# adrianstanea/UnitSpeech

Measured on AMD Instinct MI355X. Metric: mel-frames/sec @ 50 diffusion steps, 80x1024, higher is better.
Workload: dtype f32; 1 GPU; B=1 utterance(s)/GPU, 80x1024 mel, 50 diffusion steps, text+spk CFG (3 score evals/step), full-size decoder (119.1M params, synthetic weights), built-in Philox noise; batch_per_gpu=1, frames=1024, diffusion_steps=50, parallelism=utterance-sharded x1

## Files before the change

unitspeech_amd/csrc/conv_igemm.hip:

```cpp
#include <type_traits>
#include "kernels.h"
#include "pack_f16.h"

namespace us {

typedef float f32x4 __attribute__((ext_vector_type(4)));
typedef _Float16 half8 __attribute__((ext_vector_type(8)));

constexpr int TN = 128;

__device__ __forceinline__ void blds16(__amdgpu_buffer_rsrc_t rsrc, unsigned voff_bytes, unsigned soff_bytes, float* lds_dst_wave_uniform) {
  __builtin_amdgcn_raw_ptr_buffer_load_lds(rsrc, (__attribute__((address_space(3))) void*)lds_dst_wave_uniform, 16, (int)voff_bytes,
                                           (int)soff_bytes, 0, 0);
}

template <int BK, int WM, bool WINO, bool F16 = false, int NWM = 2, int NSTG = 2, bool ASPLIT = false, int NB = 2>
__global__ __launch_bounds__(NWM * 128, 2) void conv_igemm_kernel(ConvArgs a) {
  constexpr int TN = 64 * NB;
  constexpr int NW = 2 * NWM;
  constexpr int TM = NWM * WM;
  constexpr int MB = WM / 32;
  constexpr int CPR = BK / 4;
  constexpr int RPI = 64 / CPR;
  constexpr int IA = TM / RPI / NW;
  constexpr int IB = TN / RPI / NW;
  static_assert(NSTG == 2 || NSTG == 3, "two or three operand buffers");
  constexpr int SWZ_DIV = 64 / BK;
  constexpr int BUF = (TM + TN) * BK;
  extern __shared__ __attribute__((aligned(16))) float smem[];

  const int tid = threadIdx.x, lane = tid & 63;
  const int wave = __builtin_amdgcn_readfirstlane(tid >> 6);
  const int wm = wave >> 1, wn = wave & 1;
#ifdef US_LIFE
  unsigned long long life_t[5];
#define US_LIFE_AT(i) asm volatile("s_memrealtime %0\n\ts_waitcnt lgkmcnt(0)" : "=s"(life_t[i])::"memory")
  US_LIFE_AT(0);
#endif
  const int l32 = lane & 31, hh = lane >> 5;
  int bt = (int)blockIdx.x, bz = (int)blockIdx.z;
  const bool xcd_z = a.xcd_z && ((gridDim.x * gridDim.z) & 7u) == 0;
  if (xcd_z) {
    const unsigned lin = blockIdx.x + gridDim.x * blockIdx.z;
    const unsigned lp = (lin & 7u) * ((gridDim.x * gridDim.z) >> 3) + (lin >> 3);
    bz = (int)(lp / gridDim.x);
    bt = (int)(lp - (unsigned)bz * gridDim.x);
  }
  const int phase = a.nphase > 1 ? bz % a.nphase : 0;
  const int b = a.nphase > 1 ? bz / a.nphase : bz;
  const unsigned long long dy_bits = a.nphase > 1 ? a.ph_dy[phase] : a.dy_bits, dx_bits = a.nphase > 1 ? a.ph_dx[phase] : a.dx_bits,
                           wtap_bits = a.nphase > 1 ? a.ph_wtap[phase] : a.wtap_bits;
  const int a_oy0 = a.nphase > 1 ? (phase >> 1) : a.oy0, a_ox0 = a.nphase > 1 ? (phase & 1) : a.ox0;
  if (!xcd_z && (gridDim.x & 7u) == 0) bt = (bt & 7) * (int)(gridDim.x >> 3) + (bt >> 3);
  const int bx = bt / a.nt;
  const int ks = a.ksplit > 1 ? bx % a.ksplit : 0;
  const int m0 = (a.ksplit > 1 ? bx / a.ksplit : bx) * TM, n0 = (bt - bx * a.nt) * TN;
  const int Ms = a.Hs * a.Ws;
  const int nchunk = a.Cin / BK;
  const int S_all = a.ntaps * nchunk;
  const int s_lo = a.ksplit > 1 ? (int)(((long long)S_all * ks) / a.ksplit) : 0;
  const int S = a.ksplit > 1 ? (int)(((long long)S_all * (ks + 1)) / a.ksplit) - s_lo : S_all;

  const int lrow = lane / CPR, lpos = lane % CPR;
  int my[IA], mx[IA], achunk[IA];
  bool mv[IA];
#pragma unroll
  for (int j = 0; j < IA; ++j) {
    const int r = (wave * IA + j) * RPI + lrow;
    const int m = m0 + r;
    mv[j] = m < Ms;
    const int mc = mv[j] ? m : 0;
    my[j] = mc / a.Ws;
    mx[j] = mc - my[j] * a.Ws;
    achunk[j] = (lpos ^ ((r / SWZ_DIV) % CPR)) * 4;
  }
  unsigned boff[IB];
#pragma unroll
  for (int j = 0; j < IB; ++j) {
    const int r = (wave * IB + j) * RPI + lrow;
    int n = n0 + r;
    n = n < a.Cout ? n : a.Cout - 1;
    boff[j] = (unsigned)(n * BK + (lpos ^ ((r / SWZ_DIV) % CPR)) * 4) * 4u;
  }
  const unsigned a_bytes = (unsigned)a.Hin * (unsigned)a.Win * (unsigned)a.in_ld * 4u;
  const long long a_item = (long long)a.Hin * a.Win * a.in_ld;
  __amdgpu_buffer_rsrc_t rsrc_a = __builtin_amdgcn_make_buffer_rsrc((void*)(a.in + (long long)b * a_item), 0, (int)a_bytes, 0x00020000);
  __amdgpu_buffer_rsrc_t rsrc_b = __builtin_amdgcn_make_buffer_rsrc(
      (void*)(a.wt + (WINO ? 0LL : (long long)(a.wt_bdiv > 1 ? b / a.wt_bdiv : b) * a.wt_bstride)), 0, 0x7fffffff, 0x00020000);

  unsigned aoff[IA];
// ... 542 lines not shown
        stat_add(a.stats, b, n / cg, 0, bx, (double)s1);
        stat_add(a.stats, b, n / cg, 1, bx, (double)s2);
      }
    }
  }
#ifdef US_LIFE
  US_LIFE_AT(4);
  US_LIFE_AT(3);
  if (a.stamp_out && lane == 0) {
    unsigned long long* o = a.stamp_out + ((blockIdx.x + gridDim.x * blockIdx.z) * NW + wave) * 4;
    o[0] = life_t[0]; o[1] = life_t[1]; o[2] = life_t[2]; o[3] = life_t[3];
  }
#endif
}

__global__ __launch_bounds__(256) void splitk_finish_kernel(ConvArgs a) {
  __shared__ double s_g[kGroups][2];
  const int b = blockIdx.y;
  const int Ms = a.Hs * a.Ws;
  const int C4 = a.Cout >> 2;
  const long long total = (long long)Ms * C4;
  if (threadIdx.x < kGroups * 2) s_g[threadIdx.x >> 1][threadIdx.x & 1] = 0.0;
  __syncthreads();
  float t1[4] = {0.f, 0.f, 0.f, 0.f}, t2[4] = {0.f, 0.f, 0.f, 0.f};
  int tn = -1;
  const bool dense = (a.ostep == 1 && a.oy0 == 0 && a.ox0 == 0 && a.Hs == a.Hout && a.Ws == a.Wout);
  const float alpha = a.alpha ? *a.alpha : 1.f;
  float* out_b = a.out + (long long)b * a.Hout * a.Wout * a.out_ld;
  const float* add_b = a.add ? a.add + (long long)b * a.Hout * a.Wout * a.add_ld : nullptr;
  const float* om_b = a.omask ? a.omask + (long long)(b % a.omask_bmod) * a.omask_ld : nullptr;
  const long long slice = (long long)a.B * Ms * a.Cout;
  const int cg = a.Cout / kGroups;
  for (long long i = blockIdx.x * 256LL + threadIdx.x; i < total; i += (long long)gridDim.x * 256) {
    const int n = (int)(i % C4) * 4;
    const int m = (int)(i / C4);
    const float* p = a.splitk_ws + ((long long)b * Ms + m) * a.Cout + n;
    f32x4 v = *reinterpret_cast<const f32x4*>(p);
    int k = 1;
    for (; k + 8 <= a.ksplit; k += 8) {
      f32x4 u[8];
#pragma unroll
      for (int j = 0; j < 8; ++j) u[j] = *reinterpret_cast<const f32x4*>(p + (k + j) * slice);
#pragma unroll
      for (int j = 0; j < 8; ++j) v += u[j];
    }
    for (; k < a.ksplit; ++k) v += *reinterpret_cast<const f32x4*>(p + k * slice);
    if (a.bias) v += *reinterpret_cast<const f32x4*>(a.bias + n);
    if (a.stats) {
      if (tn >= 0 && tn != n) {
#pragma unroll
        for (int k = 0; k < 4; ++k) {
          atomicAdd(&s_g[(tn + k) / cg][0], (double)t1[k]);
          atomicAdd(&s_g[(tn + k) / cg][1], (double)t2[k]);
          t1[k] = t2[k] = 0.f;
        }
      }
      tn = n;
#pragma unroll
      for (int k = 0; k < 4; ++k) { t1[k] += v[k]; t2[k] += v[k] * v[k]; }
    }
    const int yy = m / a.Ws, xx = m - yy * a.Ws;
    const int ox = a.ox0 + xx * a.ostep;
    const long long pix = dense ? (long long)m : (long long)(a.oy0 + yy * a.ostep) * a.Wout + ox;
    if (a.out2) *reinterpret_cast<f32x4*>(a.out2 + ((long long)b * a.Hout * a.Wout + pix) * a.out2_ld + n) = v;
    v *= alpha;
    if (add_b) v += *reinterpret_cast<const f32x4*>(add_b + pix * a.add_ld + n);
    if (om_b) v *= om_b[ox * a.omask_step];
    *reinterpret_cast<f32x4*>(out_b + pix * a.out_ld + n) = v;
  }
  if (a.stats) {
    if (tn >= 0) {
#pragma unroll
      for (int k = 0; k < 4; ++k) {
        atomicAdd(&s_g[(tn + k) / cg][0], (double)t1[k]);
        atomicAdd(&s_g[(tn + k) / cg][1], (double)t2[k]);
      }
    }
    __syncthreads();
    if (threadIdx.x < kGroups * 2)
      stat_add(a.stats, b, threadIdx.x >> 1, threadIdx.x & 1, blockIdx.x, s_g[threadIdx.x >> 1][threadIdx.x & 1]);
  }
}

static size_t lds_bytes(int bk, int tm, int nstg = 2, int tn = TN) { return (size_t)nstg * (tm + tn) * bk * sizeof(float); }

template <int BK, int WM, bool WINO, bool F16 = false, int NWM = 2, int NSTG = 2, bool ASPLIT = false>
static hipError_t set_attr() {
  return hipFuncSetAttribute(reinterpret_cast<const void*>(&conv_igemm_kernel<BK, WM, WINO, F16, NWM, NSTG, ASPLIT>),
                             hipFuncAttributeMaxDynamicSharedMemorySize, (int)lds_bytes(BK, NWM * WM, NSTG));
}

hipError_t conv_igemm_init() {
  hipError_t e;
  if ((e = set_attr<32, 64, false>()) != hipSuccess) return e;
  if ((e = set_attr<32, 32, false>()) != hipSuccess) return e;
  if ((e = set_attr<16, 64, false>()) != hipSuccess) return e;
  if ((e = set_attr<16, 32, false>()) != hipSuccess) return e;
  if ((e = set_attr<32, 32, true>()) != hipSuccess) return e;
  if ((e = set_attr<32, 64, false, true>()) != hipSuccess) return e;
  if ((e = set_attr<32, 64, false, true, 4, 3>()) != hipSuccess) return e;
  if ((e = hipFuncSetAttribute(reinterpret_cast<const void*>(&conv_igemm_kernel<32, 64, false, true, 4, 3, false, 1>),
                               hipFuncAttributeMaxDynamicSharedMemorySize, (int)lds_bytes(32, 256, 3, 64))) != hipSuccess) return e;
  if ((e = set_attr<32, 64, false, true, 4, 3, true>()) != hipSuccess) return e;
  if ((e = set_attr<32, 64, false, true, 2, 2, true>()) != hipSuccess) return e;
  if ((e = set_attr<32, 32, false, true, 2, 2, true>()) != hipSuccess) return e;
  if ((e = set_attr<32, 32, false, true>()) != hipSuccess) return e;
  if ((e = set_attr<32, 32, true, true, 2, 3>()) != hipSuccess) return e;
  return set_attr<16, 32, true>();
}

hipError_t launch_conv_igemm(const ConvArgs& a_in, hipStream_t s) {
  ConvArgs a = a_in;
  a.range_flag = current_range_flag();
  if (a.B <= 0 || a.Hs <= 0 || a.Ws <= 0) return hipSuccess;
  if (!a.in || !a.wt || !a.out) return hipErrorInvalidValue;
  if ((a.bk != 16 && a.bk != 32) || a.Cin % a.bk != 0 || a.ntaps < 1 || a.ntaps > kMaxTaps) return hipErrorInvalidValue;
  if (a.in_ld % 4 != 0) return hipErrorInvalidValue;
  if (a.Cout % 4 != 0 || a.out_ld % 4 != 0 || (a.add && a.add_ld % 4 != 0)) return hipErrorInvalidValue;
  if ((long long)a.Hin * a.Win * a.in_ld * 4 >= (1LL << 31) || (long long)kMaxTaps * a.Cout * a.Cin * 4 >= (1LL << 31))
    return hipErrorInvalidValue;
  if (a.stats) {
    int cg = a.Cout / kGroups;
    if (a.Cout % kGroups != 0 || (cg & (cg - 1)) != 0) return hipErrorInvalidValue;
  }
  if (a.out2 && (a.out2_ld % 4 != 0 || a.wino_out || a.out_split || a.attn_part_ctx)) return hipErrorInvalidValue;
  const int Ms = a.Hs * a.Ws;
  int tn = TN;
  int nt = (a.Cout + TN - 1) / TN;
  int tm = a.tm;
  if (a.f16) {
    if (a.bk != 32) return hipErrorInvalidValue;
    if (a.f16 == 1 && !a.direct_presplit && a.ntaps == 1 && a.istride == 1 && !a.bias && !a.add) a.splitk_ws = nullptr;
    if (tm == 0) {
      if (a.f16 == 1 && (a.ntaps > 1 || a.direct_presplit)) {
        tm = (a.ntaps == 1 && a.nphase <= 1) || (long long)a.Hs * a.Ws < 512 ? 64 : 128;
      } else if (a.f16 == 1) {
        const long long per256 = (long long)((a.Hs * a.Ws + 255) / 256) * nt * a.B;
        const long long per128 = (long long)((a.Hs * a.Ws + 127) / 128) * nt * a.B;
        const long long cost256 = ((per256 + 255) / 256) * 256, cost128 = ((per128 + 255) / 256) * 128;
        constexpr int kTmModelMargin = 15;
        tm = cost128 * (100 + kTmModelMargin) < cost256 * 100 ? 128 : 256;
        if (a.Cin <= 512) tm = 128;
        constexpr int kTn64Margin = 25;
        if (a.Cout % 64 == 0 && a.Cin >= 1024 && a.Hs * a.Ws > 128) {
          const long long per64 = (long long)((a.Hs * a.Ws + 255) / 256) * ((a.Cout + 63) / 64) * a.B;
          const long long cost64 = ((per64 + 255) / 256) * 128;
          if (cost64 * (100 + kTn64Margin) < cost256 * 100) { tm = 256; tn = 64; nt = (a.Cout + 63) / 64; }
        }
      } else {
        tm = 64;
      }
    }
  }
  if (a.wino_out) {
    if (a.ntaps != 1 || a.ostep != 2 || a.istride != 1 || a.alpha) return hipErrorInvalidValue;
    if (2 * a.Hs < a.Hout || 2 * a.Ws < a.Wout) return hipErrorInvalidValue;
    tm = 64;
    a.splitk_ws = nullptr;
  }
  if (a.out_split) {
    if (a.Cout % 8 != 0 || a.out_ld % 8 != 0 || (reinterpret_cast<uintptr_t>(a.out) & 31) != 0) return hipErrorInvalidValue;
    a.splitk_ws = nullptr;
  }
  if (a.attn_part_ctx) {
    if (!((a.Cout == 3 * kHidden && a.attn_q_cols == kHidden) || (a.Cout == 2 * kHidden && a.attn_q_cols == 0)) || a.ntaps != 1 || a.istride != 1 || a.ostep != 1 || a.wino_out || a.nphase > 1 || a.bias || a.add || a.alpha ||
        a.stats || a.f16 == 1 || !a.attn_part_m || !a.attn_part_s || a.attn_nchunks != (a.Hs * a.Ws + 63) / 64)
      return hipErrorInvalidValue;
    tm = 64;
    a.splitk_ws = nullptr;
  }
  if (a.nphase > 1) {
    if (a.nphase != 4 || a.ostep != 2 || a.wino_out) return hipErrorInvalidValue;
    a.splitk_ws = nullptr;
  }
  if (tm == 0) tm = 64;
  const int mt = (Ms + tm - 1) / tm;
  const long long tiles = (long long)mt * nt * a.B;
  const int S_all = a.ntaps * (a.Cin / a.bk);
  a.ksplit = 1;
  const long long tiles_item = a.splitk_by_batch ? tiles : (long long)mt * nt;
  if (a.splitk_ws && tiles_item < 128 && S_all >= 8 && a.Cout % 4 == 0 && a.out_ld % 4 == 0 && (!a.add || a.add_ld % 4 == 0)) {
    long long k = (256 + tiles_item - 1) / tiles_item;
    if (k > S_all / 4) k = S_all / 4;
    if (k > 512 / tiles_item) k = 512 / tiles_item;
    if (k > 32) k = 32;
    if (k >= 2 && k * (long long)a.B * Ms * a.Cout <= a.splitk_ws_floats) a.ksplit = (int)k;
  }
  a.nt = nt;
  dim3 grid(mt * a.ksplit * nt, 1, a.B * (a.nphase > 1 ? a.nphase : 1));
  const size_t lds = lds_bytes(a.bk, tm);
  if (a.f16 == 2) {
    if (tm == 256) hipLaunchKernelGGL((conv_igemm_kernel<32, 64, false, true, 4, 3, true>), grid, dim3(512), lds_bytes(32, 256, 3), s, a);
    else if (tm == 128) hipLaunchKernelGGL((conv_igemm_kernel<32, 64, false, true, 2, 2, true>), grid, dim3(256), lds, s, a);
    else hipLaunchKernelGGL((conv_igemm_kernel<32, 32, false, true, 2, 2, true>), grid, dim3(256), lds, s, a);
  } else if (a.f16) {
    if (a.wino_out) hipLaunchKernelGGL((conv_igemm_kernel<32, 32, true, true, 2, 3>), grid, dim3(256), lds_bytes(32, 64, 3), s, a);
    else if (tm == 256 && tn == 64) hipLaunchKernelGGL((conv_igemm_kernel<32, 64, false, true, 4, 3, false, 1>), grid, dim3(512), lds_bytes(32, 256, 3, 64), s, a);
    else if (tm == 256) hipLaunchKernelGGL((conv_igemm_kernel<32, 64, false, true, 4, 3>), grid, dim3(512), lds_bytes(32, 256, 3), s, a);
    else if (tm == 128) hipLaunchKernelGGL((conv_igemm_kernel<32, 64, false, true>), grid, dim3(256), lds, s, a);
    else hipLaunchKernelGGL((conv_igemm_kernel<32, 32, false, true>), grid, dim3(256), lds, s, a);
  } else if (a.wino_out) {
    if (a.bk == 32)
      hipLaunchKernelGGL((conv_igemm_kernel<32, 32, true>), grid, dim3(256), lds, s, a);
    else
      hipLaunchKernelGGL((conv_igemm_kernel<16, 32, true>), grid, dim3(256), lds, s, a);
  } else if (a.bk == 32 && tm == 128)
    hipLaunchKernelGGL((conv_igemm_kernel<32, 64, false>), grid, dim3(256), lds, s, a);
  else if (a.bk == 32)
// ... 64 lines not shown
```

unitspeech_amd/csrc/decoder.hip:

```cpp
#include <hip/hip_runtime.h>

#include <cmath>
#include <cstdarg>
#include <cstdio>
#include <cstring>
#include <algorithm>
#include <map>
#include <memory>
#include <string>
#include <vector>

#include "../../include/unitspeech_hip.h"
#include "kernels.h"
#include "pack_f16.h"

using namespace us;

namespace {

thread_local std::string g_last_error;

struct DevBuf {
  float* p = nullptr;
  size_t n = 0;
// ... 5 lines not shown

struct Slot {
  std::string key;
  std::vector<int64_t> shape;
  Kind kind = Kind::RAW;
  int bk = 0;
  DevBuf buf;
  DevBuf dg;
  int bk_dg = 0;
  DevBuf wino;
  bool direct_f16 = false;
  bool wino_f16 = false;
  bool wino_dg_f16 = false;
  bool dg_f16 = false;
  int level = -1;
  DevBuf wino_dg;
  bool want_wino = false;
  DevBuf wino4;
  int wino4_form = 0;
  bool wino4_valid = false;
  bool dg_as_1x1 = false;
  bool is_qkv = false;
  DevBuf qkv_rows;
  DevBuf q_raw;
  float* grad = nullptr;
  bool grad_unscaled = false;
  bool loaded = false;
};

struct ConvW {
  Slot* w = nullptr;
  Slot* b = nullptr;
  int cin = 0, cout = 0, kh = 1, kw = 1;
};
struct ResnetW {
  int cin, cout, level;
  bool first = false;
  Slot *mlp_w, *mlp_b;
  ConvW c1, c2, res;
  Slot *g1, *b1, *g2, *b2;
  bool has_res = false;
  int index = 0;
};
struct AttnW {
  int dim, level;
  Slot* g;
  ConvW qkv;
  Slot *out_w, *out_b;
};
struct ResampleW {
  ConvW conv;
  int dim, level;
};

int pick_bk(int cin) { return (cin % 32 == 0) ? 32 : 16; }
constexpr const char* kWino4Default = "0,44,44,24";

}

namespace us {
void set_last_error(const char* msg) { g_last_error = msg ? msg : ""; }
}

struct us_decoder {
  us_config cfg{};
  int device = 0;
  std::vector<std::unique_ptr<Slot>> slots;
  std::map<std::string, Slot*> by_key;
  std::vector<int> C;
  struct Down { ResnetW r1, r2; AttnW a; bool has_ds; ResampleW ds; };
  struct Up { ResnetW r1, r2; AttnW a; ResampleW us; };
  std::vector<Down> downs;
  ResnetW mid1, mid2;
  AttnW mid_attn;
  std::vector<Up> ups;
  ConvW final_conv3;
  Slot *final_g, *final_b, *final_w1, *final_b1;
  Slot *text_uncon, *spk_uncon, *mlp0_w, *mlp0_b, *mlp2_w, *mlp2_b;
  int n_resnets = 0;
  int wino_min_level = 1;
  int wino4_level_form[8] = {0, 0, 0, 0, 0, 0, 0, 0};
  int wino_fuse = -1;
  bool wino_fuse_gn = true;
  int f16_tm = 0;
  int wgrad_side_streams = 1;
  std::vector<hipStream_t> wgrad_streams;
  std::vector<hipEvent_t> wgrad_events;
  bool training = false;
  float* zeros = nullptr;
  unsigned* range_flag = nullptr;
  unsigned* range_host = nullptr;
  bool exact = false;
  float* grad_scale = nullptr;
  CopyEnt* grad_tab_dev = nullptr;
  static constexpr size_t kLinJobs = 64;
  LinJob *lin_tab_dev = nullptr, *lin_tab_bwd_dev = nullptr;
  std::vector<CopyEnt> pending_copies;
  std::vector<PackJob> pending_packs;
  PackJob* pack_tab_dev = nullptr;
  static constexpr size_t kStageBytes = 64 << 10;
  CopyEnt* copy_tab_dev = nullptr;
  CopyEnt* copy_tab_host[4] = {nullptr, nullptr, nullptr, nullptr};
  static constexpr int kCaptureTabs = 32;
  size_t copy_tab_capture_bytes[kCaptureTabs] = {};
  CopyEnt* copy_tab_capture[kCaptureTabs] = {};
  int copy_tab_capture_used = 0;
  hipEvent_t copy_tab_ev[4] = {nullptr, nullptr, nullptr, nullptr};
  int copy_tab_i = 0;
  size_t copy_tab_cap = 0;
  std::map<uint64_t, std::shared_ptr<void>> tapes;
  uint64_t tape_serial = 0;
  static constexpr size_t kMaxTapes = 16;
  std::string err;

  struct ProfRec { hipEvent_t a, b; double flops; int kind; int f16 = 0; };
  bool prof_enabled = false;
  bool prof_active = false;
  std::vector<ProfRec> prof_pending;
  std::vector<hipEvent_t> prof_pool;
  double prof_conv_ms = 0, prof_conv_flops = 0, prof_eval_ms = 0;
  long long prof_conv_launches = 0, prof_evals = 0;
  double prof_f16_ms = 0, prof_f16_flops = 0;
  long long prof_f16_launches = 0;
  hipEvent_t prof_event() {
    if (!prof_pool.empty()) { hipEvent_t e = prof_pool.back(); prof_pool.pop_back(); return e; }
    hipEvent_t e = nullptr;
    (void)hipEventCreate(&e);
    return e;
  }

  int fail(int code, const char* fmt, ...) {
    char buf[512];
    va_list ap;
    va_start(ap, fmt);
    vsnprintf(buf, sizeof buf, fmt, ap);
    va_end(ap);
    err = buf;
    g_last_error = buf;
    return code;
  }

  Slot* add(const std::string& key, std::vector<int64_t> shape, Kind kind = Kind::RAW, int bk = 0) {
    slots.emplace_back(new Slot());
    Slot* s = slots.back().get();
    s->key = key;
    s->shape = std::move(shape);
    s->kind = kind;
    s->bk = bk;
    by_key[key] = s;
    return s;
  }

  ConvW add_conv(const std::string& p, int cout, int cin, int k, bool bias, bool transposed = false) {
    ConvW c;
    c.cin = cin; c.cout = cout; c.kh = c.kw = k;
    if (transposed)
      c.w = add(p + ".weight", {cin, cout, k, k}, Kind::CONVT_IOHW, pick_bk(cin));
    else
      c.w = add(p + ".weight", {cout, cin, k, k}, Kind::CONV_OIHW, pick_bk(cin));
    c.w->bk_dg = pick_bk(cout);
    c.b = bias ? add(p + ".bias", {cout}) : nullptr;
    return c;
  }

  ResnetW add_resnet(const std::string& p, int cin, int cout, int level) {
    ResnetW r;
// ... 223 lines not shown
  bool infer = false;
};

double* next_stats(EvalCtx& e) {
  double* p = e.b->stats + (size_t)(e.gn_slot++) * e.Bp * kGroups * kStatStride;
  return p;
}

void set_omask(EvalCtx& e, ConvArgs& a, int level_out) {
  a.omask = e.mask;
  a.omask_ld = e.T;
  a.omask_step = 1 << level_out;
  a.omask_bmod = e.Bm;
}

ConvArgs base_args(EvalCtx& e, const ConvW& w, const float* in, int in_ld, int Hin, int Win, float* out, int out_ld, int Hout,
                   int Wout) {
  ConvArgs a;
  memset(&a, 0, sizeof a);
  a.in = in; a.in_ld = in_ld;
  a.wt = w.w->buf.p;
  a.bias = w.b ? w.b->buf.p : nullptr;
  a.out = out; a.out_ld = out_ld;
  a.B = e.Bp; a.Hin = Hin; a.Win = Win; a.Cin = w.cin; a.Hout = Hout; a.Wout = Wout; a.Cout = w.cout;
  a.Hs = Hout; a.Ws = Wout; a.ostep = 1; a.istride = 1;
  a.bk = w.w->bk;
  a.f16 = w.w->direct_f16 ? 2 : 0;
  a.omask_bmod = 1;
  a.zeros = e.h->zeros;
  a.splitk_ws = e.b->splitk;
  a.splitk_by_batch = e.splitk_by_batch;
  a.splitk_ws_floats = (long long)e.b->splitk_floats;
  return a;
}

hipError_t run_conv(EvalCtx& e, const ConvArgs& a) {
  us_decoder* h = e.h;
  if (!h->prof_active) return launch_conv_igemm(a, e.s);
  us_decoder::ProfRec r;
  r.a = h->prof_event();
  r.b = h->prof_event();
  r.kind = 0;
  r.flops = 2.0 * a.B * (double)a.Hs * a.Ws * a.Cout * (double)a.Cin * a.ntaps * (a.nphase > 1 ? a.nphase : 1);
  r.f16 = a.f16 ? 1 : 0;
  (void)hipEventRecord(r.a, e.s);
  hipError_t err = launch_conv_igemm(a, e.s);
  (void)hipEventRecord(r.b, e.s);
  h->prof_pending.push_back(r);
  return err;
}

struct WinoEpi {
  const float* bias = nullptr;
  double* stats = nullptr;
  const float* add = nullptr; int add_ld = 0;
  bool mask_out = false;
};
hipError_t wino_conv(EvalCtx& e, const float* in, int in_ld, const float* U, int K, int N, int bk, int level, float* out, int out_ld,
                     const WinoEpi& ep, const WinoGnArgs* gn = nullptr, bool f16 = false, int form4 = 0, const float* U4 = nullptr) {
  const int H = e.h->cfg.n_feats >> level, W = e.T >> level;
  Buffers& b = *e.b;
  if (form4 && U4 && e.infer && !ep.add && !ep.mask_out && !(gn && gn->h_out) && (!gn || in_ld == K) &&
      (long long)H * W * in_ld * 4 < (1LL << 31) && (long long)H * W * K < (1LL << 30)) {
    int t4h, t4w;
    wino4_tiles(form4, H, W, &t4h, &t4w);
    const int nf = wino4_freqs(form4);
    hipError_t err4 = launch_wino4_input(form4, in, in_ld, b.wino_v, e.Bp, H, W, K, gn, e.s);
    if (err4 != hipSuccess) return err4;
    ConvArgs a;
    memset(&a, 0, sizeof a);
    a.f16 = 1;
    a.in = b.wino_v; a.in_ld = K;
    a.wt = U4; a.wt_bstride = (long long)N * K;
    a.Hin = t4h; a.Win = t4w; a.Cin = K; a.Cout = N;
    a.Hs = t4h; a.Ws = t4w; a.istride = 1;
    a.bk = 32;
    a.omask_bmod = 1;
    a.zeros = e.h->zeros;
    a.ntaps = 1;
    a.set_tap(0, 0, 0, 0);
    a.out = b.wino_m; a.out_ld = N;
    a.B = nf; a.Hin = a.Hs = a.Hout = e.Bp * t4h; a.Wout = t4w; a.ostep = 1;
    a.tm = e.h->f16_tm;
    a.xcd_z = K >= 256 && N >= 256;
    err4 = run_conv(e, a);
    if (err4 != hipSuccess) return err4;
    return launch_wino4_output(form4, b.wino_m, ep.bias, out, out_ld, ep.stats, e.Bp, H, W, N, e.s);
  }
  const int th = (H + 1) / 2, tw = (W + 1) / 2;
  hipError_t err = gn ? (in_ld == K ? launch_gn_wino_input(in, b.wino_v, e.Bp, H, W, K, *gn, e.s, f16) : hipErrorInvalidValue)
                      : launch_wino_input(in, in_ld, b.wino_v, e.Bp, H, W, K, e.s, f16);
  if (err != hipSuccess) return err;
  ConvArgs a;
  memset(&a, 0, sizeof a);
  a.f16 = f16 ? 1 : 0;
  a.in = b.wino_v; a.in_ld = K;
  a.wt = U; a.wt_bstride = (long long)N * K;
  a.Hin = th; a.Win = tw; a.Cin = K; a.Cout = N;
  a.Hs = th; a.Ws = tw; a.istride = 1;
  a.bk = bk;
  a.omask_bmod = 1;
  a.zeros = e.h->zeros;
  a.ntaps = 1;
  a.set_tap(0, 0, 0, 0);
  const long long fused_wgs = (long long)((th * tw + 63) / 64) * ((N + 127) / 128) * e.Bp;
  constexpr long long kFuseMinWgs = 400, kFuseMinWgsSmall = 200, kFuseSmallKN = 512 * 256;
  const long long min_wgs = (long long)K * N <= kFuseSmallKN ? kFuseMinWgsSmall : kFuseMinWgs;
  if (e.h->wino_fuse == 1 || (e.h->wino_fuse < 0 && fused_wgs >= min_wgs)) {
    a.wino_out = 1;
    a.B = e.Bp; a.Hout = H; a.Wout = W; a.ostep = 2;
    a.out = out; a.out_ld = out_ld;
    a.bias = ep.bias;
    a.stats = ep.stats;
    a.add = ep.add; a.add_ld = ep.add_ld;
    if (ep.mask_out) set_omask(e, a, level);
    us_decoder* h = e.h;
    if (!h->prof_active) return launch_conv_igemm(a, e.s);
    us_decoder::ProfRec r;
    r.a = h->prof_event(); r.b = h->prof_event(); r.kind = 0;
    r.flops = 2.0 * 16 * e.Bp * (double)th * tw * N * (double)K;
    r.f16 = a.f16 ? 1 : 0;
    (void)hipEventRecord(r.a, e.s);
    err = launch_conv_igemm(a, e.s);
    (void)hipEventRecord(r.b, e.s);
    h->prof_pending.push_back(r);
    return err;
  }
  a.out = b.wino_m; a.out_ld = N;
  a.B = 16; a.Hin = a.Hs = a.Hout = e.Bp * th; a.Wout = tw; a.ostep = 1;
  if (f16) a.tm = e.h->f16_tm;
  a.xcd_z = K >= 256 && N >= 256;
  err = run_conv(e, a);
  if (err != hipSuccess) return err;
  WinoOutExtra x{};
  x.add = ep.add; x.add_ld = ep.add_ld;
  if (ep.mask_out) { x.mask = e.mask; x.mask_ld = e.T; x.mask_step = 1 << level; x.mask_bmod = e.Bm; }
  return launch_wino_output(b.wino_m, ep.bias, out, out_ld, ep.stats, e.Bp, H, W, N, e.s, &x);
}

hipError_t conv3x3_wino(EvalCtx& e, const ConvW& w, const float* in, int in_ld, int level, float* out, int out_ld, double* stats,
                        const WinoGnArgs* gn = nullptr) {
  WinoEpi ep;
  ep.bias = w.b ? w.b->buf.p : nullptr;
  ep.stats = stats;
  const bool use4 = w.w->wino4.p && w.w->wino4_valid && w.w->wino_f16;
  return wino_conv(e, in, in_ld, w.w->wino.p, w.cin, w.cout, w.w->bk, level, out, out_ld, ep, gn, w.w->wino_f16, use4 ? w.w->wino4_form : 0,
                   use4 ? w.w->wino4.p : nullptr);
}

hipError_t conv3x3(EvalCtx& e, const ConvW& w, const float* in, int in_ld, int level, float* out, int out_ld, double* stats,
                   bool in_split = false) {
  if (w.w->wino.p && e.b->wino_v) return in_split ? hipErrorInvalidValue : conv3x3_wino(e, w, in, in_ld, level, out, out_ld, stats);
  const int H = e.h->cfg.n_feats >> level, W = e.T >> level;
  ConvArgs a = base_args(e, w, in, in_ld, H, W, out, out_ld, H, W);
  if (in_split) {
    if (a.f16 != 2) return hipErrorInvalidValue;
    a.f16 = 1;
    a.direct_presplit = 1;
  }
  a.ntaps = 9;
  for (int ky = 0; ky < 3; ++ky)
    for (int kx = 0; kx < 3; ++kx) a.set_tap(ky * 3 + kx, ky - 1, kx - 1, ky * 3 + kx);
  a.stats = stats;
  return run_conv(e, a);
}

// ... 444 lines not shown
    (void)hipEventSynchronize(h->copy_tab_ev[slot]);
  }
  memcpy(host, ents, n);
  US_HIP(h, hipMemcpyAsync(dev, host, n, hipMemcpyHostToDevice, st));
  if (cap == hipStreamCaptureStatusNone) {
    if (!h->copy_tab_ev[slot]) US_HIP(h, hipEventCreateWithFlags(&h->copy_tab_ev[slot], hipEventDisableTiming));
    US_HIP(h, hipEventRecord(h->copy_tab_ev[slot], st));
  }
  return US_OK;
}

int flush_packs(us_decoder* h, hipStream_t st) {
  const size_t n = h->pending_packs.size();
  if (n == 0) return US_OK;
  int total = 0;
  for (auto& j : h->pending_packs) { j.blk0 = total; j.nblk = pack_job_blocks(j); total += j.nblk; }
  int rc = upload_bytes(h, h->pending_packs.data(), n * sizeof(PackJob), h->pack_tab_dev, st);
  if (rc) return rc;
  RangeScope range_scope(h->range_flag);
  US_HIP(h, launch_pack_table(h->pack_tab_dev, (int)n, total, st));
  h->pending_packs.clear();
  return US_OK;
}

int flush_copies(us_decoder* h, hipStream_t st) {
  int rcp = flush_packs(h, st);
  if (rcp) return rcp;
  const size_t n = h->pending_copies.size();
  if (n == 0) return US_OK;
  int rc = upload_table(h, h->pending_copies.data(), n, h->copy_tab_dev, st);
  if (rc) return rc;
  US_HIP(h, launch_copy_table(h->copy_tab_dev, (int)n, st));
  h->pending_copies.clear();
  return US_OK;
}

int check_ready(us_decoder* h) {
  for (auto& s : h->slots)
    if (!s->loaded) return h->fail(US_EWEIGHTS, "weight '%s' has not been loaded", s->key.c_str());
  if (!h->pending_copies.empty() || !h->pending_packs.empty())
    return h->fail(US_EWEIGHTS, "us_decoder_load_weight calls have not been followed by us_decoder_flush_weights");
  return US_OK;
}

int check_shape(us_decoder* h, int Bp, int T) {
  const int q = 1 << (h->cfg.n_mults - 1);
  if (Bp <= 0 || T <= 0 || T % q != 0 || T % 4 != 0)
    return h->fail(US_EINVAL, "unsupported shape Bp=%d T=%d (T must be a positive multiple of %d)", Bp, T, q > 4 ? q : 4);
  if (h->cfg.n_feats % q != 0) return h->fail(US_EINVAL, "n_feats=%d is not divisible by %d", h->cfg.n_feats, q);
  return US_OK;
}

}

extern "C" {

int us_decoder_create(us_handle* out, const us_config* cfg) { return us_decoder_create_ex(out, cfg, 0u); }

int us_decoder_create_ex(us_handle* out, const us_config* cfg, unsigned flags) {
  if (!out || !cfg) { g_last_error = "null argument"; return US_EINVAL; }
  if (flags & ~(unsigned)US_CREATE_EXACT_FP32) { g_last_error = "unknown creation flag"; return US_EINVAL; }
  if (cfg->n_mults < 1 || cfg->n_mults > 6 || cfg->dim < 16 || cfg->dim % 16 != 0 || cfg->n_feats <= 0 || cfg->spk_emb_dim <= 0 ||
      cfg->spk_emb_dim % 4 != 0) {
    g_last_error = "unsupported configuration (dim must be a multiple of 16, 1 <= n_mults <= 6)";
    return US_EINVAL;
  }
  for (int i = 0; i < cfg->n_mults; ++i) {
    int c = cfg->dim * cfg->dim_mults[i];
    int cg = c / kGroups;
    if (cfg->dim_mults[i] < 1 || c % 16 != 0 || (cg & (cg - 1)) != 0) {
      g_last_error = "unsupported dim_mults (channels/8 must be a power of two)";
      return US_EINVAL;
    }
  }
  std::unique_ptr<us_decoder> h(new us_decoder());
  h->cfg = *cfg;
  if (hipGetDevice(&h->device) != hipSuccess) { g_last_error = "no HIP device"; return US_EHIP; }
  hipError_t e = conv_igemm_init();
  if (e != hipSuccess) { g_last_error = std::string("conv_igemm_init: ") + hipGetErrorString(e); return US_EHIP; }
  h->exact = (flags & US_CREATE_EXACT_FP32) != 0;
  if (const char* wl = getenv("US_WINO_MIN_LEVEL")) h->wino_min_level = atoi(wl);
  if (const char* wf = getenv("US_WINO_FUSE")) h->wino_fuse = atoi(wf) != 0 ? 1 : 0;
  if (const char* wf = getenv("US_WINO_FUSE_GN")) h->wino_fuse_gn = atoi(wf) != 0;
  if (const char* wt = getenv("US_F16_TM")) h->f16_tm = atoi(wt) == 64 || atoi(wt) == 128 || atoi(wt) == 256 ? atoi(wt) : 0;
  if (const char* ws = getenv("US_WGRAD_STREAM")) h->wgrad_side_streams = atoi(ws) < 0 ? 0 : (atoi(ws) > Tape::kSideMax ? Tape::kSideMax : atoi(ws));
  {
    const char* w4 = getenv("US_WINO4");
    std::string spec = w4 ? w4 : kWino4Default;
    size_t pos = 0;
    for (int l = 0; l < 8 && pos <= spec.size(); ++l) {
      const size_t comma = spec.find(',', pos);
      const std::string tok = spec.substr(pos, comma == std::string::npos ? std::string::npos : comma - pos);
      const int f = tok.empty() ? 0 : atoi(tok.c_str());
      h->wino4_level_form[l] = wino4_form_ok(f) ? f : 0;
      if (comma == std::string::npos) break;
      pos = comma + 1;
    }
    if (h->exact)
      for (int l = 0; l < 8; ++l) h->wino4_level_form[l] = 0;
  }
  h->build();
  if (hipMalloc(reinterpret_cast<void**>(&h->range_flag), 256) != hipSuccess || hipMemset(h->range_flag, 0, 256) != hipSuccess ||
      hipHostMalloc(reinterpret_cast<void**>(&h->range_host), 256) != hipSuccess ||
      hipMalloc(reinterpret_cast<void**>(&h->grad_scale), 256) != hipSuccess) {
    g_last_error = "allocation of the range word failed";
    return US_EHIP;
  }
  *h->range_host = 0u;
  {
    int max_cin = 2 * h->C.back();
    for (int c : h->C) if (2 * c > max_cin) max_cin = 2 * c;
    size_t zb = ((size_t)max_cin + 64) * sizeof(float);
    if (hipMalloc(reinterpret_cast<void**>(&h->zeros), zb) != hipSuccess || hipMemset(h->zeros, 0, zb) != hipSuccess) {
      g_last_error = "hipMalloc failed for the zero page";
      return US_EHIP;
    }
  }
  for (auto& s : h->slots) {
    bool ok = true;
    s->buf.n = numel(s->shape);
    if (!s->want_wino) {
      ok = hipMalloc(reinterpret_cast<void**>(&s->buf.p), s->buf.n * sizeof(float)) == hipSuccess;
      if (ok && (s->kind != Kind::RAW || s->dg_as_1x1)) {
        s->dg.n = s->buf.n;
        ok = hipMalloc(reinterpret_cast<void**>(&s->dg.p), s->dg.n * sizeof(float)) == hipSuccess;
      }
    }
    if (ok && s->is_qkv) {
      s->qkv_rows.n = s->buf.n;
      ok = hipMalloc(reinterpret_cast<void**>(&s->qkv_rows.p), s->qkv_rows.n * sizeof(float)) == hipSuccess;
      s->q_raw.n = (size_t)kHidden * s->shape[1];
      ok = ok && hipMalloc(reinterpret_cast<void**>(&s->q_raw.p), s->q_raw.n * sizeof(float)) == hipSuccess;
    }
    if (ok && s->want_wino) {
      s->wino.n = s->wino_dg.n = (size_t)16 * s->shape[0] * s->shape[1];
      ok = hipMalloc(reinterpret_cast<void**>(&s->wino.p), s->wino.n * sizeof(float)) == hipSuccess &&
           hipMalloc(reinterpret_cast<void**>(&s->wino_dg.p), s->wino_dg.n * sizeof(float)) == hipSuccess;
    }
    if (ok && s->dg.p && !h->exact) {
      const long long kk = s->kind == Kind::CONVT_IOHW ? s->shape[1] : s->shape[0];
      s->dg_f16 = kk % 32 == 0;
    }
    if (ok && !s->want_wino && s->kind != Kind::RAW && !h->exact) {
      const long long cin = s->kind == Kind::CONV_OIHW ? s->shape[1] : s->shape[0];
      s->direct_f16 = cin % 32 == 0;
    }
    if (ok && s->want_wino && !h->exact) {
      s->wino_f16 = s->shape[1] % 32 == 0;
      s->wino_dg_f16 = s->shape[0] % 32 == 0;
    }
    constexpr int kWino4MinK = 256;
    if (ok && s->want_wino && s->wino_f16 && s->level >= 0 && s->level < 8 && wino4_form_ok(h->wino4_level_form[s->level]) && s->shape[0] % 8 == 0 &&
        s->shape[1] >= kWino4MinK) {
      s->wino4_form = h->wino4_level_form[s->level];
      s->wino4.n = (size_t)wino4_freqs(s->wino4_form) * s->shape[0] * s->shape[1];
      ok = hipMalloc(reinterpret_cast<void**>(&s->wino4.p), s->wino4.n * sizeof(float)) == hipSuccess;
    }
    if (!ok) {
      g_last_error = "hipMalloc failed for weight store";
      for (auto& t : h->slots) { if (t->buf.p) (void)hipFree(t->buf.p); if (t->dg.p) (void)hipFree(t->dg.p); if (t->wino.p) (void)hipFree(t->wino.p); if (t->wino_dg.p) (void)hipFree(t->wino_dg.p); if (t->wino4.p) (void)hipFree(t->wino4.p); if (t->qkv_rows.p) (void)hipFree(t->qkv_rows.p); if (t->q_raw.p) (void)hipFree(t->q_raw.p); }
      return US_EHIP;
    }
  }
  h->copy_tab_cap = h->slots.size() + 8;
  if (h->copy_tab_cap * sizeof(CopyEnt) > us_decoder::kStageBytes || 3 * h->slots.size() * sizeof(PackJob) > us_decoder::kStageBytes) {
    g_last_error = "architecture too large for the weight-table staging buffers";
// ... 495 lines not shown
```

unitspeech_amd/csrc/kernels.h:

```cpp
#pragma once
#include <hip/hip_runtime.h>
#include <stdint.h>

namespace us {

#if defined(__HIPCC__)
__device__ __forceinline__ float mul_rn(float a, float b) {
#pragma clang fp contract(off)
  return a * b;
}
__device__ __forceinline__ float add_rn(float a, float b) {
#pragma clang fp contract(off)
  return a + b;
}
__device__ __forceinline__ float sub_rn(float a, float b) {
#pragma clang fp contract(off)
  return a - b;
}
typedef float f32x16 __attribute__((ext_vector_type(16)));
__device__ __forceinline__ int mfma32_row(int r, int kl) { return 8 * (r >> 2) + 4 * kl + (r & 3); }
__device__ __forceinline__ float wave_sum(float v) {
#pragma unroll
  for (int o = 32; o > 0; o >>= 1) v += __shfl_xor(v, o);
  return v;
}
double wave_sum(double) = delete;
__device__ __forceinline__ double wave_sum_d(double v) {
#pragma unroll
  for (int o = 32; o > 0; o >>= 1) v += __shfl_xor(v, o);
  return v;
}
__device__ __forceinline__ float wave_max(float v) {
#pragma unroll
  for (int o = 32; o > 0; o >>= 1) v = fmaxf(v, __shfl_xor(v, o));
  return v;
}
#endif

constexpr float kF16Over = 65520.f;
enum : unsigned {
  kRangeAct = 1u,
  kRangeWeight = 2u,
};
#if defined(__HIPCC__)
typedef _Float16 us_half;
__device__ __forceinline__ void split_f16x3(float x, us_half& hi, us_half& lo, bool& over) {
  const us_half h = (us_half)x;
  hi = h;
  lo = (us_half)((x - (float)h) * 2048.f);
  over |= fabsf(x) >= kF16Over;
}
__device__ __forceinline__ void range_report(unsigned* flag, bool over, unsigned bit) {
  if (flag && over) atomicOr(flag, bit);
}
#endif
unsigned* current_range_flag();
void set_range_flag(unsigned* p);
struct RangeScope {
  unsigned* prev;
  explicit RangeScope(unsigned* p) : prev(current_range_flag()) { set_range_flag(p); }
  ~RangeScope() { set_range_flag(prev); }
  RangeScope(const RangeScope&) = delete;
  RangeScope& operator=(const RangeScope&) = delete;
};

constexpr int kHeads = 4;
constexpr int kDimHead = 32;
constexpr int kHidden = kHeads * kDimHead;
constexpr int kGroups = 8;
constexpr int kStatSlots = 16;
constexpr int kStatStride = 2 * kStatSlots;
constexpr int kMaxTaps = 16;

struct ConvArgs {
  const float* in;
  const float* wt;
  const float* bias;
  const float* omask;
  const float* add;
  const float* alpha;
  const float* zeros;
  float* out;
  double* stats;
  long long wt_bstride;
  int xcd_z;
  int wt_bdiv;
  int in_ld, out_ld, add_ld;
  int B, Hin, Win, Cin, Hout, Wout, Cout;
  int Hs, Ws;
  int oy0, ox0, ostep;
  int istride;
  int ntaps;
  int omask_ld, omask_step, omask_bmod;
  int bk;
  int tm;
  int ksplit;
  int nt;
  int f16;
  int wino_out;
  int splitk_by_batch;
  float* splitk_ws;
  long long splitk_ws_floats;
  unsigned* range_flag;
  int direct_presplit;
  int out_split;
  float* attn_part_ctx;
  float* attn_part_m;
  float* attn_part_s;
  int attn_nchunks;
  int attn_q_cols;
  int wt_rows;
  float* out2;
  int out2_ld;
#if defined(US_STAMP) || defined(US_LIFE)
  unsigned long long* stamp_out;
#endif
  unsigned long long dy_bits, dx_bits, wtap_bits;
  void set_tap(int i, int dy, int dx, int wtap) {
    dy_bits |= (unsigned long long)(dy + 8) << (4 * i);
    dx_bits |= (unsigned long long)(dx + 8) << (4 * i);
    wtap_bits |= (unsigned long long)wtap << (4 * i);
  }
  int nphase;
  unsigned long long ph_dy[4], ph_dx[4], ph_wtap[4];
  void set_phase_tap(int ph, int i, int dy, int dx, int wtap) {
    ph_dy[ph] |= (unsigned long long)(dy + 8) << (4 * i);
    ph_dx[ph] |= (unsigned long long)(dx + 8) << (4 * i);
    ph_wtap[ph] |= (unsigned long long)wtap << (4 * i);
  }
};
#if defined(__HIPCC__)
__device__ __forceinline__ void stat_add(double* stats, long long b, int group, int which, unsigned slot, double v) {
  atomicAdd(stats + ((b * kGroups + group) * 2 + which) * kStatSlots + (slot & (kStatSlots - 1)), v);
}
__device__ __forceinline__ double stat_read(const double* stats, long long b, int group, int which) {
  const double* p = stats + ((b * kGroups + group) * 2 + which) * kStatSlots;
  double t = 0.0;
#pragma unroll
  for (int i = 0; i < kStatSlots; ++i) t += p[i];
  return t;
}
#endif
inline int qkv_src_row(int cp) {
  if (cp < kHidden) return cp;
  const int t = cp - kHidden, h = t >> 6, w = t & 63;
  return (w < kDimHead ? kHidden : 2 * kHidden) + h * kDimHead + (w & (kDimHead - 1));
}
hipError_t launch_conv_igemm(const ConvArgs& a, hipStream_t s);
hipError_t conv_igemm_init();

hipError_t launch_pack_conv_weight(const float* src, float* dst, int Cout, int Cin, int KH, int KW, bool oihw, int bk,
                                   hipStream_t s, bool qkv_rows = false);
hipError_t launch_pack_conv_weight_f16(const float* src, float* dst, int Cout, int Cin, int KH, int KW, bool oihw, hipStream_t s,
                                       bool qkv_rows = false);

hipError_t launch_first_conv(const float* in2, const float* w3, const float* b3, const float* w1, const float* b1, float* y,
                             float* r, double* stats, int Bp, int F, int T, int C, hipStream_t s);
hipError_t launch_stack_inputs(const float* x, int Bx, const float* mu, int Bmu, int n_text_uncond, const float* mu_feat,
                               const float* mask, int Bm, float* in2, int Bp, int F, int T, hipStream_t s);

hipError_t launch_gn_stats(const float* y, int ld, int B, int n, int C, double* stats, hipStream_t s);
struct GnApplyArgs {
  const float* y; int y_ld;
  const double* stats;
  const float* gamma; const float* beta;
  const float* mask; int mask_ld, mask_step, mask_bmod;
  const float* temb; int temb_ld;
  const float* res; int res_ld; int res_masked;
  const float* res2_in; const float* res2_w; const float* res2_b;
  int post_mask;
  unsigned* range_flag;
  int out_split;
  float* out; int out_ld;
  float* out2; int out2_ld;
  int B, H, W, C;
};
hipError_t launch_gn_apply(const GnApplyArgs& a, hipStream_t s);
hipError_t launch_final_conv(const float* h, int ld, const float* w, const float* b0, const float* mask, int mask_ld,
                             int mask_bmod, float* out, int B, int H, int W, int C, hipStream_t s, const double* stats = nullptr,
                             const float* gamma = nullptr, const float* beta = nullptr);

hipError_t launch_attn_ctx_partial(const float* qkv, int B, int n, float* part_ctx, float* part_m, float* part_s, int nchunks,
                                   hipStream_t s);
constexpr int kAttnMaxSplit = 16;
hipError_t launch_attn_ctx_finalize(const float* part_ctx, const float* part_m, const float* part_s, int B, int nchunks,
                                    float* ctx, float* colM, float* colS, float* split_ws, hipStream_t s);
// ... 143 lines not shown
```

Baseline: 3240 mel-frames/s.

## Add streaming weight-stationary kernel for Winograd batched GEMM with K=256

```diff
diff --git a/unitspeech_amd/csrc/conv_igemm.hip b/unitspeech_amd/csrc/conv_igemm.hip
--- a/unitspeech_amd/csrc/conv_igemm.hip
+++ b/unitspeech_amd/csrc/conv_igemm.hip
@@ -6,6 +6,7 @@
 
 typedef float f32x4 __attribute__((ext_vector_type(4)));
 typedef _Float16 half8 __attribute__((ext_vector_type(8)));
+typedef unsigned u32x4 __attribute__((ext_vector_type(4)));
 
 constexpr int TN = 128;
 
@@ -714,6 +715,146 @@
   }
 }
 
+template <int K, int NBUF>
+__global__ __launch_bounds__(512) void wino_stream_kernel(ConvArgs a, int rows, int rgroups, int total_wgs) {
+  constexpr int CPRK = K / 4;
+  constexpr int TILE_F = 32 * K;
+  constexpr int P = K / 64;
+  constexpr int NSTEP = K / 16;
+  constexpr int PSTRIDE = NSTEP / P;
+  static_assert(K == 128 || K == 256, "the B fragments of the whole K live in registers");
+  static_assert(NBUF >= 3 && (NBUF - 2) * P + 4 * (NBUF - 1) <= 63, "counted vmcnt waits");
+  extern __shared__ __attribute__((aligned(16))) float smem[];
+  const int tid = threadIdx.x, lane = tid & 63;
+  const int wave = __builtin_amdgcn_readfirstlane(tid >> 6);
+  const int l32 = lane & 31, hh = lane >> 5;
+  const unsigned per = gridDim.x >> 3;
+  const unsigned lp = (blockIdx.x & 7u) * per + (blockIdx.x >> 3);
+  if (lp >= (unsigned)total_wgs) return;
+  const int ncg = a.Cout >> 8;
+  const int rg = (int)(lp % (unsigned)rgroups);
+  const int fc = (int)(lp / (unsigned)rgroups);
+  const int f = fc / ncg, cg = fc - f * ncg;
+  const int ntile = (rows + 31) >> 5;
+  const int t_lo = ntile * rg / rgroups, t_hi = ntile * (rg + 1) / rgroups;
+  if (t_hi <= t_lo) return;
+
+  const int ncol = cg * 256 + wave * 32;
+  const int wrows = a.wt_rows ? a.wt_rows : a.Cout;
+  const float* wl = a.wt + (long long)f * a.wt_bstride + (long long)(ncol + l32) * 32 + hh * 8;
+  f32x4 bf[NSTEP][2];
+#pragma unroll
+  for (int s = 0; s < NSTEP; ++s)
+#pragma unroll
+    for (int p = 0; p < 2; ++p)
+      bf[s][p] = *reinterpret_cast<const f32x4*>(wl + (long long)(s >> 1) * wrows * 32 + (s & 1) * 16 + p * 4);
+
+  const unsigned a_bytes = (unsigned)rows * (unsigned)(K * 4);
+  const unsigned o_bytes = (unsigned)rows * (unsigned)a.Cout * 4u;
+  const __amdgpu_buffer_rsrc_t rsrc_a = __builtin_amdgcn_make_buffer_rsrc((void*)(a.in + (long long)f * rows * K), 0, (int)a_bytes, 0x00020000);
+  const __amdgpu_buffer_rsrc_t rsrc_o =
+      __builtin_amdgcn_make_buffer_rsrc((void*)(a.out + (long long)f * rows * a.Cout), 0, (int)o_bytes, 0x00020000);
+  int arow[P];
+  unsigned aoff[P];
+#pragma unroll
+  for (int j = 0; j < P; ++j) {
+    const int slot = (wave * P + j) * 64 + lane;
+    const int r = slot / CPRK, pos = slot % CPRK;
+    arow[j] = r;
+    aoff[j] = (unsigned)r * (unsigned)(K * 4) + (unsigned)((pos ^ (r & 15)) * 16);
+  }
+  auto dma_piece = [&](int tile, int buf, int j) {
+    const int m = tile * 32 + arow[j];
+    const unsigned off = (tile < t_hi && m < rows) ? (unsigned)tile * (unsigned)(32 * K * 4) + aoff[j] : a_bytes;
+    blds16(rsrc_a, off, 0u, smem + buf * TILE_F + (wave * P + j) * 256);
+  };
+
+  const int xr = l32 & 15;
+  const int a_row = l32 * K;
+  float* tr = smem + NBUF * TILE_F + wave * (32 * 36);
+  const int trow = lane >> 3, tc4 = (lane & 7) * 4;
+
+#pragma unroll
+  for (int i = 0; i < NBUF - 1; ++i)
+#pragma unroll
+    for (int j = 0; j < P; ++j) dma_piece(t_lo + i, i, j);
+
+  int cur = 0;
+  for (int t = t_lo; t < t_hi; ++t) {
+    const int nst = t - t_lo < NBUF - 1 ? t - t_lo : NBUF - 1;
+    if (nst == 0) asm volatile("s_waitcnt vmcnt(%0)" ::"n"((NBUF - 2) * P) : "memory");
+    else if (nst == 1) asm volatile("s_waitcnt vmcnt(%0)" ::"n"((NBUF - 2) * P + 4) : "memory");
+    else if (nst == 2 || NBUF == 3) asm volatile("s_waitcnt vmcnt(%0)" ::"n"((NBUF - 2) * P + 8) : "memory");
+    else asm volatile("s_waitcnt vmcnt(%0)" ::"n"((NBUF - 2) * P + 12) : "memory");
+    __builtin_amdgcn_s_barrier();
+    const int nbuf = cur == 0 ? NBUF - 1 : cur - 1;
+    const float* base = smem + cur * TILE_F + a_row;
+    f32x16 acc, total;
+#pragma unroll
+    for (int r = 0; r < 16; ++r) { acc[r] = 0.f; total[r] = 0.f; }
+    f32x4 fa[2][2];
+    auto load_frags = [&](f32x4* fr, int s) {
+#pragma unroll
+      for (int p = 0; p < 2; ++p) fr[p] = *reinterpret_cast<const f32x4*>(base + ((4 * s + 2 * hh + p) ^ xr) * 4);
+      __builtin_amdgcn_sched_barrier(0);
+    };
+    load_frags(fa[0], 0);
+#pragma unroll
+    for (int s = 0; s < NSTEP; ++s) {
+      if (s + 1 < NSTEP) load_frags(fa[(s + 1) & 1], s + 1);
+      const half8 ah = __builtin_bit_cast(half8, fa[s & 1][0]), al = __builtin_bit_cast(half8, fa[s & 1][1]);
+      const half8 bh = __builtin_bit_cast(half8, bf[s][0]), bl = __builtin_bit_cast(half8, bf[s][1]);
+      acc = __builtin_amdgcn_mfma_f32_32x32x16_f16(ah, bh, acc, 0, 0, 0);
+      if (s % PSTRIDE == 0) {
+        __builtin_amdgcn_sched_barrier(0);
+        dma_piece(t + NBUF - 1, nbuf, s / PSTRIDE);
+        __builtin_amdgcn_sched_barrier(0);
+      }
+      total = __builtin_amdgcn_mfma_f32_32x32x16_f16(ah, bl, total, 0, 0, 0);
+      total = __builtin_amdgcn_mfma_f32_32x32x16_f16(al, bh, total, 0, 0, 0);
+    }
+#pragma unroll
+    for (int r = 0; r < 16; ++r) acc[r] = __builtin_fmaf(total[r], 0x1p-11f, acc[r]);
+#pragma unroll
+    for (int r = 0; r < 16; ++r) tr[((r & 3) + 8 * (r >> 2) + 4 * hh) * 36 + l32] = acc[r];
+#pragma unroll
+    for (int k = 0; k < 4; ++k) {
+      const int dr = trow + 8 * k;
+      const int m = t * 32 + dr;
+      const f32x4 v = *reinterpret_cast<const f32x4*>(tr + dr * 36 + tc4);
+      const unsigned off = m < rows ? ((unsigned)m * (unsigned)a.Cout + (unsigned)(ncol + tc4)) * 4u : o_bytes;
+      __builtin_amdgcn_raw_buffer_store_b128(__builtin_bit_cast(u32x4, v), rsrc_o, (int)off, 0, 0);
+    }
+    cur = cur == NBUF - 1 ? 0 : cur + 1;
+  }
+  asm volatile("s_waitcnt vmcnt(0)" ::: "memory");
+}
+
+template <int K, int NBUF>
+static constexpr int stream_lds_bytes() { return (NBUF * 32 * K + 8 * 32 * 36) * (int)sizeof(float); }
+
+static bool wino_stream_route(const ConvArgs& a) {
+  if (!a.wino_stream || a.f16 != 1 || a.ntaps != 1 || a.direct_presplit || a.istride != 1 || a.tm != 0) return false;
+  if (a.bias || a.add || a.stats || a.omask || a.alpha || a.out2 || a.out_split || a.wino_out || a.attn_part_ctx || a.nphase > 1) return false;
+  if (a.Cin != 256 || a.Cout % 256 != 0 || a.in_ld != a.Cin || a.out_ld != a.Cout || a.wt_bdiv > 1) return false;
+  if (a.ostep != 1 || a.oy0 != 0 || a.ox0 != 0 || a.Hs != a.Hout || a.Ws != a.Wout || a.Hin != a.Hs || a.Win != a.Ws) return false;
+  if ((a.dy_bits & 15) != 8 || (a.dx_bits & 15) != 8 || (a.wtap_bits & 15) != 0) return false;
+  const long long rows = (long long)a.Hs * a.Ws;
+  return rows * a.Cin * 4 < (1LL << 31) && rows * a.Cout * 4 < (1LL << 31);
+}
+
+static hipError_t launch_wino_stream(const ConvArgs& a, hipStream_t s) {
+  const int rows = a.Hs * a.Ws, ntile = (rows + 31) / 32;
+  const int pairs = a.B * (a.Cout / 256);
+  int rgroups = 256 / pairs;
+  if (rgroups < 1) rgroups = 1;
+  if (rgroups > ntile) rgroups = ntile;
+  const int total = pairs * rgroups;
+  const dim3 grid(((total + 7) / 8) * 8);
+  hipLaunchKernelGGL((wino_stream_kernel<256, 3>), grid, dim3(512), (stream_lds_bytes<256, 3>()), s, a, rows, rgroups, total);
+  return hipGetLastError();
+}
+
 static size_t lds_bytes(int bk, int tm, int nstg = 2, int tn = TN) { return (size_t)nstg * (tm + tn) * bk * sizeof(float); }
 
 template <int BK, int WM, bool WINO, bool F16 = false, int NWM = 2, int NSTG = 2, bool ASPLIT = false>
@@ -738,6 +879,8 @@
   if ((e = set_attr<32, 32, false, true, 2, 2, true>()) != hipSuccess) return e;
   if ((e = set_attr<32, 32, false, true>()) != hipSuccess) return e;
   if ((e = set_attr<32, 32, true, true, 2, 3>()) != hipSuccess) return e;
+  if ((e = hipFuncSetAttribute(reinterpret_cast<const void*>(&wino_stream_kernel<256, 3>), hipFuncAttributeMaxDynamicSharedMemorySize,
+                               stream_lds_bytes<256, 3>())) != hipSuccess) return e;
   return set_attr<16, 32, true>();
 }
 
@@ -756,6 +899,7 @@
     if (a.Cout % kGroups != 0 || (cg & (cg - 1)) != 0) return hipErrorInvalidValue;
   }
   if (a.out2 && (a.out2_ld % 4 != 0 || a.wino_out || a.out_split || a.attn_part_ctx)) return hipErrorInvalidValue;
+  if (wino_stream_route(a)) return launch_wino_stream(a, s);
   const int Ms = a.Hs * a.Ws;
   int tn = TN;
   int nt = (a.Cout + TN - 1) / TN;
diff --git a/unitspeech_amd/csrc/decoder.hip b/unitspeech_amd/csrc/decoder.hip
--- a/unitspeech_amd/csrc/decoder.hip
+++ b/unitspeech_amd/csrc/decoder.hip
@@ -111,6 +111,7 @@
   int wino4_level_form[8] = {0, 0, 0, 0, 0, 0, 0, 0};
   int wino_fuse = -1;
   bool wino_fuse_gn = true;
+  bool wino_stream = true;
   int f16_tm = 0;
   int wgrad_side_streams = 1;
   std::vector<hipStream_t> wgrad_streams;
@@ -500,6 +501,7 @@
     a.out = b.wino_m; a.out_ld = N;
     a.B = nf; a.Hin = a.Hs = a.Hout = e.Bp * t4h; a.Wout = t4w; a.ostep = 1;
     a.tm = e.h->f16_tm;
+    a.wino_stream = e.h->wino_stream ? 1 : 0;
     a.xcd_z = K >= 256 && N >= 256;
     err4 = run_conv(e, a);
     if (err4 != hipSuccess) return err4;
@@ -1110,6 +1112,7 @@
   if (const char* wl = getenv("US_WINO_MIN_LEVEL")) h->wino_min_level = atoi(wl);
   if (const char* wf = getenv("US_WINO_FUSE")) h->wino_fuse = atoi(wf) != 0 ? 1 : 0;
   if (const char* wf = getenv("US_WINO_FUSE_GN")) h->wino_fuse_gn = atoi(wf) != 0;
+  if (const char* ws = getenv("US_WINO_STREAM")) h->wino_stream = atoi(ws) != 0;
   if (const char* wt = getenv("US_F16_TM")) h->f16_tm = atoi(wt) == 64 || atoi(wt) == 128 || atoi(wt) == 256 ? atoi(wt) : 0;
   if (const char* ws = getenv("US_WGRAD_STREAM")) h->wgrad_side_streams = atoi(ws) < 0 ? 0 : (atoi(ws) > Tape::kSideMax ? Tape::kSideMax : atoi(ws));
   {
diff --git a/unitspeech_amd/csrc/kernels.h b/unitspeech_amd/csrc/kernels.h
--- a/unitspeech_amd/csrc/kernels.h
+++ b/unitspeech_amd/csrc/kernels.h
@@ -102,6 +102,7 @@
   float* splitk_ws;
   long long splitk_ws_floats;
   unsigned* range_flag;
+  int wino_stream;
   int direct_presplit;
   int out_split;
   float* attn_part_ctx;
```

Result: faster. 3305 mel-frames/s (median of 6 runs) (+2.0%).
